# ffreyer/MonteCarlo.jl

Measured on AMD Instinct MI355X. Metric: DQMC sweeps/sec, 16x16 Hubbard beta=8 dtau=0.1; achieved % fp64 MFMA roofline, higher is better.
Workload: dtype f64

## Files before the change

montecarlo.jl_amd/csrc/engine.cpp:

```cpp
#include <hip/hip_runtime.h>

#include <algorithm>
#include <cmath>
#include <cstdio>
#include <cstdlib>
#include <cstring>
#include <string>
#include <vector>

#include "../../include/dqmc_hip.h"
#include "kernels.h"
#include "state_blob.h"
#include <rccl/rccl.h>

using namespace dqmc;

struct dqmc_comm {
    ncclComm_t comm = nullptr;
    int nranks = 1, rank = 0, device = 0;
};

static thread_local std::string g_create_error;

struct UTStack;
// ... 463 lines not shown
    auto apply = [&](int op, const double *F) {
        for (int c = 0; c < n; ++c) {
            const double *m = M.data() + (size_t)n * c;
            double *t = T.data() + (size_t)n * c;
            for (int y = 0; y < 16; ++y)
                for (int x = 0; x < 16; ++x) {
                    double acc = 0.0;
                    for (int k = 0; k < 16; ++k) {
                        const double f = F[(op == 0 ? x : y) + 16 * k];
                        const int src = op == 0 ? k + 16 * y : op == 1 ? x + 16 * k : op == 2 ? ((x - y + k) & 15) + 16 * k
                                                                                               : ((x + y - k) & 15) + 16 * k;
                        acc += f * m[src];
                    }
                    t[x + 16 * y] = acc;
                }
        }
        M.swap(T);
    };
    const double *F[4] = {fx, fy, fd, fa};
    static const int orders[5][4] = {{3, 2, 0, 1}, {1, 2, 3, 0}, {0, 2, 3, 1}, {0, 3, 2, 1}, {1, 3, 2, 0}};
    double emax = 0.0, rmax = 0.0;
    for (size_t i = 0; i < (size_t)n * n; ++i) emax = std::max(emax, std::fabs(E[i]));
    for (const auto &ord : orders) {
        std::fill(M.begin(), M.end(), 0.0);
        for (int i = 0; i < n; ++i) M[i + (size_t)n * i] = 1.0;
        for (int k = 0; k < 4; ++k) apply(ord[k], F[ord[k]]);
        for (size_t i = 0; i < (size_t)n * n; ++i) {
            const double r = std::fabs(E[i] - M[i]);
            if (!(r <= rmax)) rmax = r;
        }
    }
    return std::isfinite(emax) && std::isfinite(rmax) && rmax <= 256.0 * 2.220446049250313e-16 * emax;
}

static void read_kernel_switches(dqmc_handle *h)
{
    KernelSwitches &k = h->sw;
    k.qr_noblocked = getenv("DQMC_QR_NOBLOCKED") != nullptr;
    if (const char *e = getenv("DQMC_QRB_SITES")) k.qrb_sites = atoi(e) & 7;
    if (const char *e = getenv("DQMC_QR_TAIL")) k.qr_tail = atoi(e) != 0;
    k.qr_sc1 = getenv("DQMC_QR_SC1") != nullptr;
    k.qr_nocoop = getenv("DQMC_QR_NOCOOP") != nullptr;
    if (const char *e = getenv("DQMC_QR_FORCE_TIMEOUT"))
        k.qr_force_timeout = strncmp(e, "step:", 5) == 0 ? 2 + atoi(e + 5) : (strncmp(e, "extra:", 6) == 0 ? 1000 + atoi(e + 6) : 1);
    k.qr_nopanel = getenv("DQMC_QR_NOPANEL") != nullptr;
    k.trsm_simple = getenv("DQMC_TRSM_SIMPLE") != nullptr;
    k.sweep_split = getenv("DQMC_SWEEP_SPLIT") != nullptr;
    k.flush_ncp2 = getenv("DQMC_FLUSH_NCP2") != nullptr;
    k.no_slab = getenv("DQMC_NO_SLAB") != nullptr;
    k.no_kron = getenv("DQMC_NO_KRON") != nullptr;
    k.no_wrap_flush = getenv("DQMC_NO_WRAP_FLUSH") != nullptr;
    k.wrap_two_launch = getenv("DQMC_WRAP_TWO_LAUNCH") != nullptr;
    k.tdm_general = getenv("DQMC_TDM_GENERAL") != nullptr;
}

static int padded_units(const dqmc_handle *h) { return (h->units + 7) / 8 * 8; }
static bool udt_blocked_fits(const dqmc_handle *h, int per_cu) { return per_cu >= 1 && padded_units(h) * 8 <= h->cus * per_cu; }
static bool sweep_fused_fits(const dqmc_handle *h)
{
    const int ncp = (h->n % 256 == 0) ? 2 : 1, nt = (h->n % 128 == 0) ? 8 : 4;
    const int flush_blocks = padded_units(h) * (h->n / 64) * (h->n / (16 * nt * ncp));
    return h->W + flush_blocks <= h->cus;
}

static int alloc_qr_workspace(dqmc_handle *h)
{
    CHK(dalloc(h, &h->qr_ws.errflag, (size_t)1));
    h->qr_ws.tail = h->sw.qr_tail;
    h->qr_ws.force_sc1 = h->sw.qr_sc1;
    h->qr_ws.no_coop = h->sw.qr_nocoop;
    h->qr_ws.no_panel = h->sw.qr_nopanel;
    h->qr_ws.force_timeout = h->sw.qr_force_timeout;
    if (h->n > 256) return 0;
    hipDeviceProp_t prop;
    HIPCHK(hipGetDeviceProperties(&prop, h->p.device_id));
    h->cus = prop.multiProcessorCount;
    const size_t slots = (size_t)((h->units + 7) / 8) * 8 * QR_COOP_SLOTS_PER_UNIT;
    CHK(dalloc(h, &h->qr_ws.mailbox, slots * QR_COOP_SLOT));
    CHK(dalloc(h, &h->qr_ws.fb, (size_t)2));
    h->qr_ws.max_blocks = h->cus * qr_coop_blocks_per_cu();
    h->qr_ws.epoch = 0;
    h->qrb_sites = 0;
    if (h->n == 256 && !h->sw.qr_noblocked) {
        const int per_cu = qrb_blocks_per_cu();
        if (udt_blocked_fits(h, per_cu)) {
            CHK(dalloc(h, (char **)&h->qr_ws.mailbox2, qrb_mailbox_bytes(h->units)));
            h->qr_ws.blk_max_blocks = h->cus * per_cu;
            h->qrb_sites = h->sw.qrb_sites;
        }
    }
    return 0;
}
static int alloc_wrap_handoff(dqmc_handle *h)
{
    if (!h->kron || h->n != 256 || h->rect || h->sw.wrap_two_launch) return 0;
    hipDeviceProp_t prop;
    HIPCHK(hipGetDeviceProperties(&prop, h->p.device_id));
    h->cus = prop.multiProcessorCount;
    for (int pf = 0; pf < 2; ++pf) h->wrap_blocks[pf] = h->cus * kron_wrap_blocks_per_cu(pf != 0);
    if (kron_wrap_grid(h->units) > std::max(h->wrap_blocks[0], h->wrap_blocks[1])) return 0;
    return dalloc(h, &h->wrap_cnt, (size_t)kron_wrap_grid(h->units) / 16 * KR_CNT_STRIDE);
}
static bool wrap_one_launch(const dqmc_handle *h, bool pending)
{
    return h->wrap_cnt && h->n == 256 && !h->tri && !h->rect && kron_wrap_grid(h->units) <= h->wrap_blocks[pending ? 1 : 0];
}
// ... 28 lines not shown
        Timed t(h, DQMC_K_QR);
        HIPCHK(launch_qr_pivot(n, h->units, A, h->nn, q.tau, q.pivot, &h->qr_ws, q.W, h->nn, &F, h->stream, q.V, h->nn));
    }
    {
        Timed t(h, DQMC_K_MISC);
        HIPCHK(launch_udt_finish(n, h->units, A, h->nn, F, h->nn, q.pivot, Dout, n, q.V, h->nn, Tout, h->nn, apply,
                                 h->stream));
    }
    return 0;
}
static int udt_formq(dqmc_handle *h, double *Uout, QrSet &q)
{
    const int n = h->n;
    GemmArgs g = gemm_base(h, U_(h, q.V), 1, U_(h, q.V), 0, q.S);
    g.tri = (n % 64 == 0) ? 1 : 0;
    CHK(run_gemm(h, g));
    {
        Timed t(h, DQMC_K_TRSM);
        HIPCHK(launch_trsm_right_upper(n, h->units, q.V, h->nn, q.S, h->nn, nullptr, q.tau, n, q.W, h->nn, q.winv, h->sw, h->stream, q.ts));
    }
    g = gemm_base(h, U_(h, q.W), 0, U_(h, q.V), 1, Uout);
    g.alpha = -1.0;
    g.ident = 1.0;
    g.tri = (n % 64 == 0) ? 2 : 0;
    CHK(run_gemm(h, g));
    return 0;
}
static bool udt_is_fused(const dqmc_handle *h, int site) { return (h->qrb_sites >> site) & 1; }
static int udt_fused(dqmc_handle *h, const double *A, double *Uout, double *Dout, double *Tout, int apply, QrSet &q,
                     const double *B = nullptr)
{
    Timed t(h, DQMC_K_QR);
    HIPCHK(launch_udt_blocked(h->units, A, h->nn, Uout, h->nn, Dout, h->n, Tout, h->nn, q.pivot, &h->qr_ws, apply, h->stream, B,
                              h->nn));
    return 0;
}
static int udt(dqmc_handle *h, double *A, double *Uout, double *Dout, double *Tout, int apply)
{
    if (udt_is_fused(h, 0) && Tout && Tout != A) return udt_fused(h, A, Uout, Dout, Tout, apply, h->qs);
    CHK(udt_factor(h, A, Dout, Tout, apply, h->qs));
    return udt_formq(h, Uout, h->qs);
}
static int rdivp_set(dqmc_handle *h, const double *A, const double *T, double *Out, const QrSet &q)
{
    Timed t(h, DQMC_K_TRSM);
    HIPCHK(launch_trsm_right_upper(h->n, h->units, A, h->nn, T, h->nn, q.pivot, nullptr, 0, Out, h->nn, q.winv, h->sw, h->stream, q.ts));
    return 0;
}
static int rdivp(dqmc_handle *h, double *A, const double *T)
{
    return rdivp_set(h, A, T, A, h->qs);
}

static int calculate_greens_src(dqmc_handle *h, double *out, Udt L, Udt R, double *a2_copy = nullptr)
{
    const int n = h->n;
    QrSet &q = h->qs;
    GemmArgs g = gemm_base(h, U_(h, L.t), 0, U_(h, R.t), 1, out);
    g.colscale = vs_arr(R.d, n);
    g.rowscale = vs_arr(L.d, n);
    CHK(run_gemm(h, g));
    if (udt_is_fused(h, 1)) {
        if (L.u == h->Tl) return fail(h, DQMC_ERR_STATE, "calculate_greens: Ul aliases Tl");
        CHK(udt_fused(h, out, h->Tl, h->Dr, q.W, 0, q, L.u));
        CHK(rdivp_set(h, R.u, q.W, h->Ur, q));
    } else {
        CHK(udt_factor(h, out, h->Dr, nullptr, 0, q));
        CHK(rdivp_set(h, R.u, out, h->Ur, q));
        CHK(udt_formq(h, h->Tr, q));
        CHK(run_gemm(h, gemm_base(h, U_(h, L.u), 0, U_(h, h->Tr), 0, h->Tl)));
    }
    g = gemm_base(h, U_(h, h->Tl), 1, U_(h, h->Ur), 0, h->Tr);
    g.adddiag = vs_arr(h->Dr, n);
    CHK(run_gemm(h, g));
    if (a2_copy) CHK(copy_mat(h, a2_copy, h->Tr));
    const double *tlul = h->Tr;
    if (udt_is_fused(h, 2)) {
        CHK(udt_fused(h, h->Tr, h->Ul, h->Dr, q.W, 0, q, h->Tl));
        CHK(rdivp_set(h, h->Ur, q.W, h->Ur, q));
        tlul = h->Ul;
    } else {
        CHK(udt_factor(h, h->Tr, h->Dr, nullptr, 0, q));
        CHK(rdivp_set(h, h->Ur, h->Tr, h->Ur, q));
        CHK(udt_formq(h, h->Ul, q));
        CHK(run_gemm(h, gemm_base(h, U_(h, h->Tl), 0, U_(h, h->Ul), 0, h->Tr)));
    }
    g = gemm_base(h, U_(h, h->Ur), 0, U_(h, tlul), 1, out);
    g.kscale = vs_inv(h->Dr, n);
    CHK(run_gemm(h, g));
    return 0;
}
static int calculate_greens(dqmc_handle *h, double *out, double *a2_copy = nullptr)
{
    return calculate_greens_src(h, out, Udt{h->Ul, h->Dl, h->Tl}, Udt{h->Ur, h->Dr, h->Tr}, a2_copy);
}

enum { CB_LEFT_B = 0, CB_LEFT_BINV = 1, CB_LEFT_BDAG = 2, CB_RIGHT_B = 3, CB_RIGHT_BINV = 4, CB_RIGHT_ET = 5,
       CB_LEFT_ETINV = 6 };
static int cb_mult(dqmc_handle *h, int which, int slice, const double *X, double *O, const double *qscale)
{
    CbArgs a{};
    a.n = h->n; a.nb = h->nb; a.kmax = h->cb.kmax;
    a.side = (which == CB_RIGHT_B || which == CB_RIGHT_BINV || which == CB_RIGHT_ET) ? 1 : 0;
    a.seq_len = h->cb.len[which];
    for (int i = 0; i < a.seq_len; ++i) a.seq[i] = h->cb.seq[which][i];
    a.vals = h->cb.vals; a.cols = h->cb.cols;
    a.X = X; a.O = O; a.strideX = h->nn;
    a.conf = slice >= 1 ? h->conf + (long)(slice - 1) * h->N : nullptr;
    a.conf_stride = (long)h->N * h->M;
    a.epl = h->epl; a.eml = h->eml;
    switch (which) {
    case CB_LEFT_B: a.pre_conf = +1; a.pre_vec = h->cb.mu; break;
    case CB_LEFT_BINV: a.post_conf = -1; a.post_vec = h->cb.mu_inv; break;
    case CB_LEFT_BDAG: a.post_conf = +1; a.post_vec = h->cb.mu; break;
    case CB_RIGHT_B: a.post_conf = +1; a.post_vec = h->cb.mu; break;
    case CB_RIGHT_BINV: a.pre_conf = -1; a.pre_vec = h->cb.mu_inv; break;
    default: break;
    }
    a.qscale = qscale; a.qstride = h->n;
    hipEvent_t ea, eb;
    timing_events(h, &ea, &eb);
    HIPCHK(launch_cb_apply(a, h->units, h->stream, ea, eb));
    return timing_push(h, ea, eb, DQMC_K_GEMM);
}

static SlabArgs slab_base(dqmc_handle *h, const double *X0, long x_su, long x_sb, double *out)
{
    SlabArgs a{};
    a.n_units = h->units; a.nb = h->nb; a.nsteps = 0;
    a.X0 = X0; a.x_su = x_su; a.x_sb = x_sb;
    a.out = out; a.out_su = h->nn;
    a.conf_stride = (long)h->N * h->M;
    a.epl = h->epl; a.eml = h->eml;
    return a;
}
static void slab_step_const(dqmc_handle *h, SlabArgs &a, const double *C)
{
    SlabStep &st = a.st[a.nsteps++];
    st = SlabStep{};
    st.A = C; st.su = 0; st.sb = h->nn;
}
static void slab_step_unit(dqmc_handle *h, SlabArgs &a, const double *A)
// ... 191 lines not shown
    const int8_t *c = conf_slice(h, curr_slice);
    SlabArgs a = slab_base(h, h->eTinv2, 0, h->nn, dst);
    slab_step_unit(h, a, src);
    a.st[0].pre_conf = c; a.st[0].pre_sign = -1;
    slab_step_const(h, a, h->eT2);
    a.st[1].pre_conf = c; a.st[1].pre_sign = +1;
    return run_slab(h, a);
}
static int wrap_greens_inplace(dqmc_handle *h, double *gf, int curr_slice, int direction);
static int wrap_greens(dqmc_handle *h, double **gf, int curr_slice, int direction)
{
    if (oop_wrap(h)) {
        CHK(wrap_greens_slab(h, *gf, h->tmp1, curr_slice, direction));
        std::swap(*gf, h->tmp1);
        return 0;
    }
    return wrap_greens_inplace(h, *gf, curr_slice, direction);
}
static int wrap_greens_inplace(dqmc_handle *h, double *gf, int curr_slice, int direction)
{
    if (h->cb.on) {
        const int l = direction == -1 ? curr_slice - 1 : curr_slice;
        CHK(cb_mult(h, direction == -1 ? CB_LEFT_BINV : CB_LEFT_B, l, gf, gf, nullptr));
        CHK(cb_mult(h, direction == -1 ? CB_RIGHT_B : CB_RIGHT_BINV, l, gf, gf, nullptr));
        return 0;
    }
    if (direction == -1) {
        const int l = curr_slice - 1;
        GemmArgs g = gemm_base(h, C_(h, h->eTinv2), 0, U_(h, gf), 0, h->tmp1);
        g.rowscale = vs_conf(h, l, -1);
        CHK(run_gemm(h, g));
        g = gemm_base(h, U_(h, h->tmp1), 0, C_(h, h->eT2), 0, gf);
        g.colscale = vs_conf(h, l, +1);
        CHK(run_gemm(h, g));
    } else {
        const int l = curr_slice;
        GemmArgs g = gemm_base(h, C_(h, h->eT2), 0, U_(h, gf), 0, h->tmp1);
        g.kscale = vs_conf(h, l, +1);
        CHK(run_gemm(h, g));
        g = gemm_base(h, U_(h, h->tmp1), 0, C_(h, h->eTinv2), 0, gf);
        g.kscale = vs_conf(h, l, -1);
        CHK(run_gemm(h, g));
    }
    return 0;
}

static int reset_slot(dqmc_handle *h, int slot)
{
    const int sp = h->K + 1;
    CHK(set_identity(h, uslot(h, sp)));
    CHK(set_ones(h, dslot(h, sp)));
    CHK(set_identity(h, tslot(h, sp)));
    slot_swap_spare(h, slot);
    return 0;
}
static int prop_check(dqmc_handle *h)
{
    Timed t(h, DQMC_K_MISC);
    HIPCHK(launch_prop_check(h->n, h->nb, h->W, h->greens_temp, h->greens, h->nn, h->stats, h->pc_scratch, h->stream));
    return 0;
}

static int init_stack(dqmc_handle *h)
{
    CHK(set_identity(h, h->Ul)); CHK(set_identity(h, h->Ur));
    CHK(set_identity(h, h->Tl)); CHK(set_identity(h, h->Tr));
    CHK(set_ones(h, h->Dl)); CHK(set_ones(h, h->Dr));
    h->current_slice = 0;
    h->direction = 0;
    return 0;
}
static int build_stack(dqmc_handle *h)
{
    CHK(reset_slot(h, 0));
    for (int i = 1; i <= h->K; ++i) CHK(add_slice_sequence_left(h, i));
    h->current_slice = h->M + 1;
    h->direction = -1;
    return 0;
}

static int propagate(dqmc_handle *h)
{
    const int M = h->M, s = h->s;
    if (h->direction == 1) {
        if (h->current_slice % s == 0) {
            h->current_slice += 1;
            if (h->current_slice == 1) {
                const Udt R = slot_ref(h, 0);
                CHK(reset_slot(h, 0));
                discard_pending_flush(h);
                CHK(calculate_greens_src(h, h->greens, slot_ref(h, 0), R));
            } else if (1 < h->current_slice && h->current_slice <= M) {
                const int idx = (h->current_slice - 1) / s;
                const Udt R = slot_ref(h, idx);
                const bool wt = h->p.check_propagation_error != 0, wt_slab = wt && oop_wrap(h);
                CHK(add_slice_sequence_left(h, idx, wt_slab));
                const Udt L = slot_ref(h, idx);
                if (wt && !wt_slab) {
                    CHK(materialize_pending_flush(h));
                    CHK(copy_mat(h, h->greens_temp, h->greens));
                    CHK(wrap_greens(h, &h->greens_temp, h->current_slice - 1, 1));
                }
                if (wt_slab) {
                    std::swap(h->greens, h->greens_alt);
                    CHK(calculate_greens_src(h, h->greens, L, R));
                    CHK(prop_check(h));
                    return 0;
                }
                discard_pending_flush(h);
                CHK(calculate_greens_src(h, h->greens, L, R));
                if (h->p.check_propagation_error) CHK(prop_check(h));
            } else {
                CHK(add_slice_sequence_left(h, h->K));
                h->direction = -1;
                h->current_slice = M + 1;
                CHK(propagate(h));
            }
        } else {
            CHK(wrap_greens(h, &h->greens, h->current_slice, 1));
            h->current_slice += 1;
        }
    } else {
        if ((h->current_slice - 1) % s == 0) {
            h->current_slice -= 1;
            if (h->current_slice == M) {
                const Udt L = slot_ref(h, h->K);
                CHK(reset_slot(h, h->K));
                discard_pending_flush(h);
                CHK(calculate_greens_src(h, h->greens, L, slot_ref(h, h->K)));
                CHK(wrap_greens(h, &h->greens, h->current_slice + 1, -1));
            } else if (0 < h->current_slice && h->current_slice < M) {
                const int idx = h->current_slice / s + 1;
                const Udt L = slot_ref(h, idx - 1);
                CHK(add_slice_sequence_right(h, idx));
                const Udt R = slot_ref(h, idx - 1);
                if (h->p.check_propagation_error) {
                    CHK(materialize_pending_flush(h));
                    std::swap(h->greens_temp, h->greens);
                }
                discard_pending_flush(h);
                CHK(calculate_greens_src(h, h->greens, L, R));
                if (h->p.check_propagation_error) CHK(prop_check(h));
                CHK(wrap_greens(h, &h->greens, h->current_slice + 1, -1));
            } else {
                CHK(add_slice_sequence_right(h, 1));
                h->direction = 1;
                h->current_slice = 0;
                CHK(propagate(h));
            }
        } else {
            CHK(wrap_greens(h, &h->greens, h->current_slice, -1));
            h->current_slice -= 1;
        }
    }
    return 0;
}

static int sweep_spatial_launches(dqmc_handle *h);
static bool sweep_takes_fused(const dqmc_handle *h) { return h->sweep_fused && h->n % 64 == 0 && h->N >= 128; }
static int sweep_spatial(dqmc_handle *h)
{
    const int l = h->current_slice;
    if (l < 1 || l > h->M) return fail(h, DQMC_ERR_STATE, "sweep_spatial: current_slice outside 1..slices");
    CHK(sweep_spatial_launches(h));
    return 0;
}
static int sweep_spatial_launches(dqmc_handle *h)
{
    const int l = h->current_slice;
    int8_t *cslice = h->conf + (long)(l - 1) * h->N;
    h->conf_version++;
    CHK(materialize_pending_flush(h));
    double *cur = h->greens, *alt = h->greens_alt;
    const size_t istr = (size_t)h->units * sweep_lu_image_doubles();

    const long cstr = (long)h->N * h->M;
    hipEvent_t a, b;
    if (sweep_takes_fused(h)) {
        const int nc = h->N / 64;
        timing_events(h, &a, &b);
        HIPCHK(launch_sweep_lu(h->n, h->nb, h->W, cur, h->nn, cslice, cstr, 0, 64, h->lu_img, h->sc, h->rng, h->stats,
                               h->p.check_sign_problem, h->qr_ws.errflag, h->stream, a, b));
        CHK(timing_push(h, a, b, DQMC_K_SWEEP));
        for (int c = 1; c < nc; ++c) {
            timing_events(h, &a, &b);
            HIPCHK(launch_sweep_fused(h->n, h->nb, h->W, cur, alt, h->nn, cslice, cstr, 64 * c, 64 * (c - 1),
                                      h->lu_img + (size_t)(c & 1) * istr, h->lu_img + (size_t)((c - 1) & 1) * istr, h->sc,
                                      h->rng, h->stats, h->p.check_sign_problem, h->qr_ws.errflag, h->stream, a, b));
            CHK(timing_push(h, a, b, DQMC_K_SWEEP));
            std::swap(cur, alt);
        }
        const double *img_last = h->lu_img + (size_t)((nc - 1) & 1) * istr;
        if (fold_wrap_flush(h)) {
            h->pf = dqmc_handle::PendingFlush{cur, img_last, 64 * (nc - 1)};
        } else {
// ... 1395 lines not shown
```

montecarlo.jl_amd/csrc/kernels.h:

```cpp
#pragma once
#include <hip/hip_runtime.h>
#include <stdint.h>

namespace dqmc {

struct VecSrc {
    int mode;
    const double *d;
    long stride;
    const int8_t *conf;
    long conf_stride;
    double cpos[2], cneg[2];
};
static inline VecSrc vs_none() { VecSrc v = {}; v.mode = 0; return v; }
static inline VecSrc vs_arr(const double *d, long stride) { VecSrc v = {}; v.mode = 1; v.d = d; v.stride = stride; return v; }
static inline VecSrc vs_inv(const double *d, long stride) { VecSrc v = {}; v.mode = 3; v.d = d; v.stride = stride; return v; }
static inline VecSrc vs_min1(const double *d, long stride) { VecSrc v = {}; v.mode = 4; v.d = d; v.stride = stride; return v; }
static inline VecSrc vs_maxinv(const double *d, long stride) { VecSrc v = {}; v.mode = 5; v.d = d; v.stride = stride; return v; }
#ifdef __HIPCC__
__device__ __forceinline__ double vs_get(const VecSrc &v, int unit, int nb, int i)
{
    if (v.mode == 1) return v.d[(long)unit * v.stride + i];
    if (v.mode == 3) return 1.0 / v.d[(long)unit * v.stride + i];
    if (v.mode == 2) {
// ... 43 lines not shown
    const int8_t *col_conf; int col_sign;
    long conf_stride;
    double epl, eml;
};
hipError_t launch_slab_chain(const SlabArgs &a, hipStream_t s, hipEvent_t start = nullptr, hipEvent_t stop = nullptr);
struct KronStep {
    const double *ax, *ay;
    const int8_t *pre_conf; int pre_sign;
    const int8_t *post_conf; int post_sign;
};
struct KronArgs {
    int n_units, nb, nsteps;
    KronStep st[SLAB_MAX_STEPS];
    const double *X0; long x_su;
    double *out; long out_su;
    const double *col_d; long col_stride;
    int transpose_out;
    long conf_stride;
    double epl, eml;
    const double *pf_img; long pf_img_su;
    int pf_site0;
    double *wrap_out;
    unsigned *wrap_cnt; unsigned wrap_target;
    int *errflag;
};
hipError_t launch_kron_chain(const KronArgs &a, hipStream_t s, hipEvent_t start = nullptr, hipEvent_t stop = nullptr);
constexpr int KR_CNT_STRIDE = 32;
inline int kron_wrap_grid(int n_units) { return (n_units + 7) / 8 * 8 * 16; }
int kron_wrap_blocks_per_cu(bool pending);
hipError_t launch_kron_wrap(const KronArgs &a, hipStream_t s, hipEvent_t start = nullptr, hipEvent_t stop = nullptr);
hipError_t launch_kron3_chain(const KronArgs &a, hipStream_t s, hipEvent_t start = nullptr, hipEvent_t stop = nullptr);
hipError_t launch_tri_chain(const KronArgs &a, hipStream_t s, hipEvent_t start = nullptr, hipEvent_t stop = nullptr);
hipError_t launch_ttp_chain(const KronArgs &a, hipStream_t s, hipEvent_t start = nullptr, hipEvent_t stop = nullptr);
constexpr int BILAYER_FB = 264;
hipError_t launch_bilayer_chain(const KronArgs &a, hipStream_t s, hipEvent_t start = nullptr, hipEvent_t stop = nullptr);
hipError_t launch_rect_chain(const KronArgs &a, hipStream_t s, hipEvent_t start = nullptr, hipEvent_t stop = nullptr);

struct KernelSwitches {
    bool qr_noblocked = false;
    int qrb_sites = 7;
    bool qr_tail = true;
    bool qr_sc1 = false;
    bool qr_nocoop = false;
    int qr_force_timeout = 0;
    bool qr_nopanel = false;
    bool trsm_simple = false;
    bool sweep_split = false;
    bool flush_ncp2 = false;
    bool no_slab = false;
    bool no_kron = false;
    bool no_wrap_flush = false;
    bool wrap_two_launch = false;
    bool tdm_general = false;
};

constexpr int QR_COOP_SLOT = 528;
constexpr int QR_COOP_SLOTS_PER_UNIT = 16;
struct QrCoopWorkspace {
    double *mailbox = nullptr;
    int *errflag = nullptr;
    int *fb = nullptr;
    unsigned long long epoch = 0;
    int max_blocks = 0;
    bool tail = true;
    int force_sc1 = 0;
    int no_coop = 0;
    bool no_panel = false;
    int force_timeout = 0;
    double *mailbox2 = nullptr;
    int blk_max_blocks = 0;
};
hipError_t launch_udt_blocked(int n_units, const double *A, long strideA, double *U, long strideU, double *D, long strideD,
                              double *T, long strideT, int *pivot, QrCoopWorkspace *ws, int apply_pivot, hipStream_t s,
                              const double *B = nullptr, long strideB = 0);
size_t qrb_mailbox_bytes(int n_units);
int qrb_blocks_per_cu();
hipError_t launch_qr_pivot(int n, int n_units, double *A, long strideA, double *tau, int *pivot,
                           QrCoopWorkspace *ws, double *W, long strideW, const double **factored, hipStream_t s,
                           double *X = nullptr, long strideX = 0);
int qr_coop_blocks_per_cu();
int qr_coop_grid(int n, int n_units, const QrCoopWorkspace *ws);

hipError_t launch_udt_finish(int n, int n_units, double *A, long strideA, const double *F, long strideF,
                             const int *pivot, double *D, long strideD, double *V, long strideV, double *Tout,
                             long strideT, int apply_pivot, hipStream_t s);

hipError_t launch_trsm_right_upper(int n, int n_units, const double *A, long strideA, const double *T,
                                   long strideT, const int *pivot, const double *dmul, long strideV,
                                   double *Out, long strideOut, double *winv, const KernelSwitches &sw,
                                   hipStream_t s, double *scratch = nullptr);

struct SweepConsts {
    double gamma[2], ebos[2], dup[2], ddn[2];
};
struct WalkerRng {
    unsigned long long seed;
    unsigned long long draw;
    const double *uniforms;
    unsigned long long n_uniforms;
    int exhausted;
};
struct DevMagStats { double max, min, sum; long long count; };
struct DevStats {
    long long prop_local, acc_local;
    DevMagStats negative_probability, propagation_error;
};
#ifdef __HIPCC__
__device__ __forceinline__ double philox_uniform(unsigned long long seed, unsigned long long index)
{
    unsigned int c0 = (unsigned int)index, c1 = (unsigned int)(index >> 32), c2 = 0u, c3 = 0u;
    unsigned int k0 = (unsigned int)seed, k1 = (unsigned int)(seed >> 32);
#pragma unroll
    for (int r = 0; r < 10; ++r) {
        const unsigned long long p0 = (unsigned long long)0xD2511F53u * c0;
        const unsigned long long p1 = (unsigned long long)0xCD9E8D57u * c2;
        const unsigned int n0 = (unsigned int)(p1 >> 32) ^ c1 ^ k0;
        const unsigned int n1 = (unsigned int)p1;
        const unsigned int n2 = (unsigned int)(p0 >> 32) ^ c3 ^ k1;
        const unsigned int n3 = (unsigned int)p0;
        c0 = n0; c1 = n1; c2 = n2; c3 = n3;
        k0 += 0x9E3779B9u;
        k1 += 0xBB67AE85u;
    }
    const unsigned long long hi = c0 >> 5, lo = c1 >> 6;
    return (double)((hi << 26) | lo) * (1.0 / 9007199254740992.0);
}

__device__ __forceinline__ double philox4_uniform(unsigned long long seed, unsigned int c0, unsigned int c1,
                                                  unsigned int c2, unsigned int c3)
{
    unsigned int k0 = (unsigned int)seed, k1 = (unsigned int)(seed >> 32);
#pragma unroll
    for (int r = 0; r < 10; ++r) {
        const unsigned long long p0 = (unsigned long long)0xD2511F53u * c0;
        const unsigned long long p1 = (unsigned long long)0xCD9E8D57u * c2;
        const unsigned int n0 = (unsigned int)(p1 >> 32) ^ c1 ^ k0;
        const unsigned int n1 = (unsigned int)p1;
        const unsigned int n2 = (unsigned int)(p0 >> 32) ^ c3 ^ k1;
        const unsigned int n3 = (unsigned int)p0;
        c0 = n0; c1 = n1; c2 = n2; c3 = n3;
        k0 += 0x9E3779B9u;
        k1 += 0xBB67AE85u;
    }
// ... 199 lines not shown
```

montecarlo.jl_amd/csrc/qr.hip:

```cpp
#include "kernels.h"
#include <cstdlib>

namespace dqmc {

__device__ __forceinline__ double wave_sum(double x)
{
#pragma unroll
    for (int off = 32; off > 0; off >>= 1) x += __shfl_xor(x, off, 64);
    return x;
}

constexpr int QR_THREADS = 1024;
constexpr int QR_WAVES = QR_THREADS / 64;

template <int QMAX, int QR_UC>
__global__ __launch_bounds__(QR_THREADS) void qr_pivot_kernel(int n, double *__restrict__ Aall, long strideA,
                                                             double *__restrict__ tauall,
                                                             int *__restrict__ pivall,
                                                             const double *__restrict__ srcall, long strideSrc,
                                                             int *guard, int guard_val)
{
    extern __shared__ __attribute__((aligned(16))) double sm[];
    if (guard && guard[0] != guard_val) return;
    if (srcall) {
// ... 1686 lines not shown
}

__global__ __launch_bounds__(16) void trsm_diag_inv_kernel(int n, const double *__restrict__ Tall, long sT,
                                                          const double *__restrict__ dmulall, long sV,
                                                          double *__restrict__ Wall, int nblk)
{
    __shared__ double B[16][17], rdg[16];
    const int J = blockIdx.x, unit = blockIdx.y, j = threadIdx.x, j0 = J << 4;
    const double *__restrict__ T = Tall + (long)unit * sT;
    const double *__restrict__ dmul = dmulall ? dmulall + (long)unit * sV : nullptr;
    double *__restrict__ W = Wall + ((long)unit * nblk + J) * 256;
    const int col = j0 + j;
    {
        const int cc = min(col, n - 1);
        double bv[16], dv;
#pragma unroll
        for (int i = 0; i < 16; ++i) bv[i] = T[min(j0 + i, n - 1) + (long)n * cc];
        dv = dmul ? dmul[cc] : T[cc + (long)n * cc];
        asm volatile("" ::: "memory");
#pragma unroll
        for (int i = 0; i < 16; ++i) B[i][j] = (col < n && j0 + i < n && i < j) ? bv[i] : 0.0;
        rdg[j] = col < n ? (dmul ? dv : 1.0 / dv) : 1.0;
    }
    __syncthreads();
    double wcol[16];
#pragma unroll
    for (int i = 15; i >= 0; --i) {
        double sum = (i == j) ? 1.0 : 0.0;
#pragma unroll
        for (int kk = i + 1; kk < 16; ++kk) sum -= B[i][kk] * ((kk <= j) ? wcol[kk] : 0.0);
        wcol[i] = (i <= j) ? sum * rdg[i] : 0.0;
    }
#pragma unroll
    for (int i = 0; i < 16; ++i) W[i + 16 * j] = wcol[i];
}

__global__ void trsm_gather_kernel(int n, const double *__restrict__ Aall, long sA, const int *__restrict__ pivall,
                                   double *__restrict__ Wall, long sW)
{
    const int unit = blockIdx.y;
    const double *__restrict__ A = Aall + (long)unit * sA;
    double *__restrict__ W = Wall + (long)unit * sW;
    const int *__restrict__ piv = pivall ? pivall + (long)unit * n : nullptr;
    const long nn = (long)n * n;
    for (long idx = blockIdx.x * (long)blockDim.x + threadIdx.x; idx < nn; idx += (long)gridDim.x * blockDim.x) {
        const int r = (int)(idx % n), c = (int)(idx / n);
        W[idx] = A[r + (long)n * (piv ? piv[c] : c)];
    }
}

hipError_t launch_trsm_rl(int nr, int nc, int c0, int ld, int nblk_all, int n_units, const double *A, long sA,
                          const double *T, long sT, const int *pivot, double *Out, long sO, const double *winv,
                          hipStream_t s);

hipError_t launch_trsm_right_upper(int n, int n_units, const double *A, long sA, const double *T, long sT,
                                   const int *pivot, const double *dmul, long sV, double *Out, long sO,
                                   double *winv, const KernelSwitches &sw, hipStream_t s, double *scratch)
{
    const bool no_mfma = sw.trsm_simple;
    if (n <= 256 && winv && !no_mfma) {
        const int nblk = (n + 15) / 16;
        hipLaunchKernelGGL(trsm_diag_inv_kernel, dim3(nblk, n_units), dim3(16), 0, s, n, T, sT, dmul, sV, winv, nblk);
        return launch_trsm_rl(n, n, 0, n, nblk, n_units, A, sA, T, sT, pivot, Out, sO, winv, s);
    }
    if (n > 256 && winv && scratch && sA == sO && !no_mfma) {
        const int nblk = (n + 15) / 16;
        int pw = 256;
        for (int cand = 256; cand >= 128; cand -= 16)
            if (n % cand == 0) { pw = cand; break; }
        hipLaunchKernelGGL(trsm_diag_inv_kernel, dim3(nblk, n_units), dim3(16), 0, s, n, T, sT, dmul, sV, winv, nblk);
        int bx = (int)(((long)n * n + 255) / 256);
        if (bx > 128) bx = 128;
        hipLaunchKernelGGL(trsm_gather_kernel, dim3(bx, n_units), dim3(256), 0, s, n, A, sA, pivot, scratch, sO);
        for (int c0 = 0; c0 < n; c0 += pw) {
            const int nc = n - c0 < pw ? n - c0 : pw;
            if (c0 > 0) {
                GemmArgs g{};
                g.M = n; g.N = nc; g.K = c0;
                g.n_units = n_units; g.nb = 1;
                g.A = mat(scratch, sO, n);
                g.B = mat(T + (long)n * c0, sT, n);
                g.C = scratch + (long)n * c0; g.strideC = sO; g.ldc = n;
                g.kscale = g.colscale = g.rowscale = g.adddiag = vs_none();
                g.alpha = -1.0; g.ident = 0.0; g.beta = 1;
                hipError_t e = launch_gemm(g, s);
                if (e != hipSuccess) return e;
            }
            hipError_t er = launch_trsm_rl(n, nc, c0, n, nblk, n_units, scratch, sO, T, sT, nullptr, scratch, sO, winv, s);
            if (er != hipSuccess) return er;
        }
        hipError_t e = hipMemcpyAsync(Out, scratch, sizeof(double) * (size_t)n_units * sO, hipMemcpyDeviceToDevice, s);
        if (e != hipSuccess) return e;
        return hipGetLastError();
    }
    const size_t budget = 150 * 1024;
    auto need = [&](int rs) { return ((size_t)n * rs + ((n + 63) & ~63) + 256) * sizeof(double); };
    int rs = 64;
    while (rs > 16 && need(rs) > budget) rs >>= 1;
    if (need(rs) > budget) return hipErrorInvalidValue;
    const int slabs = (n + rs - 1) / rs;
    dim3 grid(n_units * slabs), block(256);
    const size_t lds = need(rs);
#define TR_LAUNCH(RS)                                                                                         \
    do {                                                                                                      \
        (void)hipFuncSetAttribute((const void *)trsm_kernel<RS>, hipFuncAttributeMaxDynamicSharedMemorySize, (int)lds); \
        hipLaunchKernelGGL((trsm_kernel<RS>), grid, block, lds, s, n, A, sA, T, sT, pivot, dmul, sV, Out, sO, slabs); \
// ... 10 lines not shown
```

montecarlo.jl_amd/csrc/trsm_rl.hip:

```cpp
#include "kernels.h"
#include <type_traits>

namespace dqmc {

typedef double d4_t __attribute__((ext_vector_type(4)));

#ifdef TR_STAMPS
__device__ long long *tr_stamp_ptr = nullptr;
#define TR_STAMP(idx)                                                                                        \
    do {                                                                                                     \
        if (blockIdx.x == 0 && (threadIdx.x & 63) == 0 && tr_stamp_ptr)                                      \
            tr_stamp_ptr[(threadIdx.x >> 6) * 64 + (idx)] = (long long)__builtin_amdgcn_s_memtime();         \
    } while (0)
#else
#define TR_STAMP(idx) do { } while (0)
#endif
constexpr int TR_TS = 18;
template <bool FULLB>
__global__ __launch_bounds__(256) void trsm_rl_kernel(int nr, int n, int c0, int ld, int nblk_all,
                                                     const double *__restrict__ Aall, long sA,
                                                     const double *__restrict__ Tall, long sT,
                                                     const int *__restrict__ pivall, double *__restrict__ Oall, long sO,
                                                     int slabs, const double *__restrict__ Wall, int n_units)
{
    extern __shared__ __attribute__((aligned(16))) double trl_sm[];
    double (*Tl)[256 * TR_TS] = reinterpret_cast<double (*)[256 * TR_TS]>(trl_sm);
    double (*Xi)[2][4 * 64] = reinterpret_cast<double (*)[2][4 * 64]>(trl_sm + 3 * 256 * TR_TS);
    double (*Wl)[4 * 64] = reinterpret_cast<double (*)[4 * 64]>(trl_sm + 3 * 256 * TR_TS + 2 * 2 * 256);
    const int bid = blockIdx.x, xcd = bid & 7, seq = bid >> 3;
    const int unit = (seq / slabs) * 8 + xcd, row0 = (seq % slabs) * 32;
    if (unit >= n_units) return;
    const double *__restrict__ A = Aall + (long)unit * sA;
    const double *__restrict__ T = Tall + (long)unit * sT + (long)ld * c0 + c0;
    const int *__restrict__ piv = pivall ? pivall + (long)unit * ld : nullptr;
    double *__restrict__ O = Oall + (long)unit * sO;
    const int tid = threadIdx.x, lane = tid & 63, w = tid >> 6, g = lane >> 4, ci = lane & 15;
    const int rt = w & 1, par = w >> 1;
    const int nblk = FULLB ? 16 : (n + 15) >> 4;
    const double *__restrict__ Wu = Wall + ((long)unit * nblk_all + (c0 >> 4)) * 256;
    const int row = row0 + 16 * rt + ci;
    const int rowc = min(row, nr - 1);

    TR_STAMP(0);
    d4_t x[8];
    int pjv[8][4];
#pragma unroll
    for (int t = 0; t < 8; ++t)
#pragma unroll
        for (int r = 0; r < 4; ++r) {
            const int cc = min(16 * (2 * t + par) + 4 * r + g, n - 1);
            pjv[t][r] = piv ? piv[c0 + cc] : c0 + cc;
        }
#pragma unroll
    for (int t = 0; t < 8; ++t)
#pragma unroll
        for (int r = 0; r < 4; ++r) x[t][r] = A[(unsigned)(rowc + ld * pjv[t][r])];
    asm volatile("" ::: "memory");
#pragma unroll
    for (int t = 0; t < 8; ++t) {
        const int L = 2 * t + par;
#pragma unroll
        for (int r = 0; r < 4; ++r) {
            const int col = 16 * L + 4 * r + g;
            x[t][r] = (L < nblk && col < n && row < nr) ? x[t][r] : 0.0;
        }
    }
#ifdef TR_STAMPS
    TR_STAMP(40);
    asm volatile("s_waitcnt vmcnt(0)" ::: "memory");
    TR_STAMP(41);
#endif
    constexpr int TR_RING = 3;
    double pv[TR_RING][16];
    auto request = [&](auto Jc) {
        constexpr int J = decltype(Jc)::value, S = J % TR_RING;
        if (J >= nblk) return;
        const int k = FULLB ? 16 * J + (tid & 15) : min(16 * J + (tid & 15), n - 1);
#pragma unroll
        for (int i = (FULLB ? J + 1 : 0); i < 16; ++i) {
            const int c = FULLB ? (tid >> 4) + 16 * i : min((tid >> 4) + 16 * i, n - 1);
            pv[S][i] = T[(unsigned)(ld * c + k)];
        }
    };
    auto deposit = [&](auto Jc) {
        constexpr int J = decltype(Jc)::value, S = J % TR_RING;
        if (J >= nblk) return;
        double *tl = Tl[J % 3];
        const int k = tid & 15;
#pragma unroll
        for (int i = (FULLB ? J + 1 : 0); i < 16; ++i) {
            const int c = (tid >> 4) + 16 * i;
            const bool live = FULLB || (c < n && c >= 16 * (J + 1) && 16 * J + k < n);
            tl[c * TR_TS + k] = live ? pv[S][i] : 0.0;
        }
    };
    auto finish = [&](auto Jc) {
        constexpr int J = decltype(Jc)::value, t_own = J >> 1;
        d4_t o = {0.0, 0.0, 0.0, 0.0};
#pragma unroll
        for (int q = 0; q < 4; ++q) o = __builtin_amdgcn_mfma_f64_16x16x4f64(Wl[J][q * 64 + lane], x[t_own][q], o, 0, 0, 0);
#pragma unroll
        for (int r = 0; r < 4; ++r) {
            Xi[J & 1][rt][r * 64 + lane] = o[r];
            const int col = 16 * J + 4 * r + g;
            if (FULLB || (row < nr && col < n)) O[(unsigned)(row + ld * (c0 + col))] = o[r];
        }
    };
#define TRL_IC(K) std::integral_constant<int, (K)>{}
    request(TRL_IC(0));
    request(TRL_IC(1));
    request(TRL_IC(2));
    {
        const int q = tid >> 6, l = tid & 63, src = (4 * q + (l >> 4)) + 16 * (l & 15);
        double wv[16];
#pragma unroll
        for (int J = 0; J < 16; ++J) wv[J] = Wu[(unsigned)((FULLB ? J : min(J, nblk - 1)) * 256 + src)];
#pragma unroll
        for (int J = 0; J < 16; ++J) Wl[J][tid] = wv[J];
    }
#ifdef TR_STAMPS
    TR_STAMP(42);
    asm volatile("s_waitcnt vmcnt(0)" ::: "memory");
    TR_STAMP(43);
#endif
    deposit(TRL_IC(0));
    TR_STAMP(44);
    __syncthreads();
    TR_STAMP(1);
    if (par == 0) finish(TRL_IC(0));
    deposit(TRL_IC(1));
    request(TRL_IC(3));
    asm volatile("s_waitcnt lgkmcnt(0)\n\ts_barrier" ::: "memory");
    auto step = [&](auto Jc) {
        constexpr int J = decltype(Jc)::value;
        if (!FULLB && J >= nblk) return;
        const double *xi = Xi[J & 1][rt];
        const double *tl = Tl[J % 3];
        const double b0 = -xi[lane], b1 = -xi[64 + lane], b2 = -xi[128 + lane], b3 = -xi[192 + lane];
        auto body = [&](auto pc) {
            constexpr int PAR = decltype(pc)::value;
            constexpr bool own_next = J + 1 < 16 && ((J + 1) & 1) == PAR;
            constexpr int t_next = (J + 1) >> 1;
            if constexpr (own_next) {
                if (FULLB || J + 1 < nblk) {
                    const double *ta = tl + (16 * (J + 1) + ci) * TR_TS + g;
                    x[t_next] = __builtin_amdgcn_mfma_f64_16x16x4f64(ta[0], b0, x[t_next], 0, 0, 0);
                    x[t_next] = __builtin_amdgcn_mfma_f64_16x16x4f64(ta[4], b1, x[t_next], 0, 0, 0);
                    x[t_next] = __builtin_amdgcn_mfma_f64_16x16x4f64(ta[8], b2, x[t_next], 0, 0, 0);
                    x[t_next] = __builtin_amdgcn_mfma_f64_16x16x4f64(ta[12], b3, x[t_next], 0, 0, 0);
                    finish(TRL_IC(J + 1 < 16 ? J + 1 : 15));
                }
            }
            constexpr int t_first = own_next ? t_next + 1 : (J + 2 - PAR) / 2;
            const double bq[4] = {b0, b1, b2, b3};
#pragma unroll
            for (int q = 0; q < 4; ++q)
#pragma unroll
                for (int t = t_first; t < 8; ++t) {
                    if (!FULLB && 2 * t + PAR >= nblk) continue;
                    const double *ta = tl + (16 * (2 * t + PAR) + ci) * TR_TS + g;
                    x[t] = __builtin_amdgcn_mfma_f64_16x16x4f64(ta[4 * q], bq[q], x[t], 0, 0, 0);
                }
        };
        if (par == 0) body(TRL_IC(0));
        else body(TRL_IC(1));
        deposit(TRL_IC(J + 2));
        request(TRL_IC(J + 4));
        TR_STAMP(2 + 2 * J);
        asm volatile("s_waitcnt lgkmcnt(0)\n\ts_barrier" ::: "memory");
        TR_STAMP(3 + 2 * J);
    };
#define TRL_STEP(K) step(std::integral_constant<int, K>{})
    TRL_STEP(0); TRL_STEP(1); TRL_STEP(2); TRL_STEP(3); TRL_STEP(4); TRL_STEP(5); TRL_STEP(6); TRL_STEP(7);
    TRL_STEP(8); TRL_STEP(9); TRL_STEP(10); TRL_STEP(11); TRL_STEP(12); TRL_STEP(13); TRL_STEP(14); TRL_STEP(15);
#undef TRL_STEP
#undef TRL_IC
    TR_STAMP(34);
}
#ifdef TR_STAMPS
extern "C" int dqmc_debug_tr_stamps(void *devptr)
{
    return (int)hipMemcpyToSymbol(HIP_SYMBOL(tr_stamp_ptr), &devptr, sizeof(void *));
}
#endif

hipError_t launch_trsm_rl(int nr, int nc, int c0, int ld, int nblk_all, int n_units, const double *A, long sA,
                          const double *T, long sT, const int *pivot, double *Out, long sO, const double *winv,
                          hipStream_t s)
{
    if (nc > 256 || nc < 1) return hipErrorInvalidValue;
    const size_t lds_r = (3 * 256 * TR_TS + 2 * 2 * 256 + 16 * 256) * sizeof(double);
    int dev = 0;
    (void)hipGetDevice(&dev);
    static unsigned attr_mask = 0;
    if (!(attr_mask & (1u << dev))) {
        (void)hipFuncSetAttribute((const void *)trsm_rl_kernel<true>, hipFuncAttributeMaxDynamicSharedMemorySize, (int)lds_r);
        (void)hipFuncSetAttribute((const void *)trsm_rl_kernel<false>, hipFuncAttributeMaxDynamicSharedMemorySize, (int)lds_r);
        attr_mask |= 1u << dev;
    }
    const int slabs = (nr + 31) / 32;
    const int groups = (n_units + 7) / 8;
    if (nc == 256 && nr % 32 == 0)
        hipLaunchKernelGGL(trsm_rl_kernel<true>, dim3(groups * 8 * slabs), dim3(256), lds_r, s, nr, nc, c0, ld, nblk_all, A, sA, T,
                           sT, pivot, Out, sO, slabs, winv, n_units);
    else
        hipLaunchKernelGGL(trsm_rl_kernel<false>, dim3(groups * 8 * slabs), dim3(256), lds_r, s, nr, nc, c0, ld, nblk_all, A, sA,
                           T, sT, pivot, Out, sO, slabs, winv, n_units);
    return hipGetLastError();
}

}
```

Baseline: 821.1.

## Fuse right triangular solve with final Green's product and propagation check

For n=256, the last rdivp triangular solve of calculate_greens is fused with the closing GEMM (Ur·diag(1/D)·(TlUl)^T) and, when requested, the propagation-error check, all in one kernel. The solved slab stays in registers and LDS instead of being written to Ur and read back by a separate GEMM and check kernel. This removes two launches and a full matrix round trip per Green's function. The cost is a more complex kernel with extra register pressure, and a product phase that reuses the T-panel LDS region.

```diff
diff --git a/montecarlo.jl_amd/csrc/engine.cpp b/montecarlo.jl_amd/csrc/engine.cpp
--- a/montecarlo.jl_amd/csrc/engine.cpp
+++ b/montecarlo.jl_amd/csrc/engine.cpp
@@ -539,6 +539,8 @@
     k.no_wrap_flush = getenv("DQMC_NO_WRAP_FLUSH") != nullptr;
     k.wrap_two_launch = getenv("DQMC_WRAP_TWO_LAUNCH") != nullptr;
     k.tdm_general = getenv("DQMC_TDM_GENERAL") != nullptr;
+    k.no_rdivp_product = getenv("DQMC_NO_RDIVP_PRODUCT") != nullptr;
+    k.no_rdivp_check = getenv("DQMC_NO_RDIVP_CHECK") != nullptr;
 }
 
 static int padded_units(const dqmc_handle *h) { return (h->units + 7) / 8 * 8; }
@@ -673,7 +675,18 @@
     return rdivp_set(h, A, T, A, h->qs);
 }
 
-static int calculate_greens_src(dqmc_handle *h, double *out, Udt L, Udt R, double *a2_copy = nullptr)
+static int prop_check(dqmc_handle *h, const double *A, const double *B)
+{
+    Timed t(h, DQMC_K_MISC);
+    HIPCHK(launch_prop_check(h->n, h->nb, h->W, A, B, h->nn, h->stats, h->pc_scratch, h->stream));
+    return 0;
+}
+static bool rdivp_product_on(const dqmc_handle *h)
+{
+    return h->n == 256 && !h->sw.no_rdivp_product && !h->sw.trsm_simple && h->qs.winv;
+}
+static int calculate_greens_src(dqmc_handle *h, double *out, Udt L, Udt R, double *a2_copy = nullptr,
+                                const double *check = nullptr)
 {
     const int n = h->n;
     QrSet &q = h->qs;
@@ -696,19 +709,38 @@
     CHK(run_gemm(h, g));
     if (a2_copy) CHK(copy_mat(h, a2_copy, h->Tr));
     const double *tlul = h->Tr;
+    const double *t2 = h->Tr;
+    const bool fused = rdivp_product_on(h);
     if (udt_is_fused(h, 2)) {
         CHK(udt_fused(h, h->Tr, h->Ul, h->Dr, q.W, 0, q, h->Tl));
-        CHK(rdivp_set(h, h->Ur, q.W, h->Ur, q));
+        if (!fused) CHK(rdivp_set(h, h->Ur, q.W, h->Ur, q));
         tlul = h->Ul;
+        t2 = q.W;
+    } else if (fused) {
+        CHK(udt_factor(h, h->Tr, h->Dr, nullptr, 0, q));
+        CHK(udt_formq(h, h->Ul, q));
+        CHK(run_gemm(h, gemm_base(h, U_(h, h->Tl), 0, U_(h, h->Ul), 0, q.W)));
+        tlul = q.W;
     } else {
         CHK(udt_factor(h, h->Tr, h->Dr, nullptr, 0, q));
         CHK(rdivp_set(h, h->Ur, h->Tr, h->Ur, q));
         CHK(udt_formq(h, h->Ul, q));
         CHK(run_gemm(h, gemm_base(h, U_(h, h->Tl), 0, U_(h, h->Ul), 0, h->Tr)));
     }
+    if (fused) {
+        const bool in_launch = check && !h->sw.no_rdivp_check;
+        {
+            Timed t(h, DQMC_K_TRSM);
+            HIPCHK(launch_rdivp_product(n, h->units, h->Ur, h->nn, t2, h->nn, q.pivot, q.winv, tlul, h->nn, h->Dr, n, out, h->nn,
+                                        in_launch ? check : nullptr, h->stats, h->pc_scratch, h->nb, h->stream));
+        }
+        if (check && !in_launch) CHK(prop_check(h, check, out));
+        return 0;
+    }
     g = gemm_base(h, U_(h, h->Ur), 0, U_(h, tlul), 1, out);
     g.kscale = vs_inv(h->Dr, n);
     CHK(run_gemm(h, g));
+    if (check) CHK(prop_check(h, check, out));
     return 0;
 }
 static int calculate_greens(dqmc_handle *h, double *out, double *a2_copy = nullptr)
@@ -1006,12 +1038,6 @@
     CHK(set_ones(h, dslot(h, sp)));
     CHK(set_identity(h, tslot(h, sp)));
     slot_swap_spare(h, slot);
-    return 0;
-}
-static int prop_check(dqmc_handle *h)
-{
-    Timed t(h, DQMC_K_MISC);
-    HIPCHK(launch_prop_check(h->n, h->nb, h->W, h->greens_temp, h->greens, h->nn, h->stats, h->pc_scratch, h->stream));
     return 0;
 }
 
@@ -1057,13 +1083,11 @@
                 }
                 if (wt_slab) {
                     std::swap(h->greens, h->greens_alt);
-                    CHK(calculate_greens_src(h, h->greens, L, R));
-                    CHK(prop_check(h));
+                    CHK(calculate_greens_src(h, h->greens, L, R, nullptr, h->greens_temp));
                     return 0;
                 }
                 discard_pending_flush(h);
-                CHK(calculate_greens_src(h, h->greens, L, R));
-                if (h->p.check_propagation_error) CHK(prop_check(h));
+                CHK(calculate_greens_src(h, h->greens, L, R, nullptr, h->p.check_propagation_error ? h->greens_temp : nullptr));
             } else {
                 CHK(add_slice_sequence_left(h, h->K));
                 h->direction = -1;
@@ -1093,8 +1117,7 @@
                     std::swap(h->greens_temp, h->greens);
                 }
                 discard_pending_flush(h);
-                CHK(calculate_greens_src(h, h->greens, L, R));
-                if (h->p.check_propagation_error) CHK(prop_check(h));
+                CHK(calculate_greens_src(h, h->greens, L, R, nullptr, h->p.check_propagation_error ? h->greens_temp : nullptr));
                 CHK(wrap_greens(h, &h->greens, h->current_slice + 1, -1));
             } else {
                 CHK(add_slice_sequence_right(h, 1));
diff --git a/montecarlo.jl_amd/csrc/kernels.h b/montecarlo.jl_amd/csrc/kernels.h
--- a/montecarlo.jl_amd/csrc/kernels.h
+++ b/montecarlo.jl_amd/csrc/kernels.h
@@ -119,6 +119,8 @@
     bool no_wrap_flush = false;
     bool wrap_two_launch = false;
     bool tdm_general = false;
+    bool no_rdivp_product = false;
+    bool no_rdivp_check = false;
 };
 
 constexpr int QR_COOP_SLOT = 528;
@@ -156,6 +158,12 @@
                                    long strideT, const int *pivot, const double *dmul, long strideV,
                                    double *Out, long strideOut, double *winv, const KernelSwitches &sw,
                                    hipStream_t s, double *scratch = nullptr);
+
+struct DevStats;
+hipError_t launch_rdivp_product(int n, int n_units, const double *A, long strideA, const double *T, long strideT,
+                                const int *pivot, double *winv, const double *B, long strideB, const double *D,
+                                long strideD, double *C, long strideC, const double *Gt, DevStats *stats,
+                                unsigned long long *pc_scratch, int nb, hipStream_t s);
 
 struct SweepConsts {
     double gamma[2], ebos[2], dup[2], ddn[2];
diff --git a/montecarlo.jl_amd/csrc/qr.hip b/montecarlo.jl_amd/csrc/qr.hip
--- a/montecarlo.jl_amd/csrc/qr.hip
+++ b/montecarlo.jl_amd/csrc/qr.hip
@@ -1762,6 +1762,19 @@
 hipError_t launch_trsm_rl(int nr, int nc, int c0, int ld, int nblk_all, int n_units, const double *A, long sA,
                           const double *T, long sT, const int *pivot, double *Out, long sO, const double *winv,
                           hipStream_t s);
+
+hipError_t launch_trsm_rl_product(int n_units, const double *A, long sA, const double *T, long sT, const int *pivot,
+                                  const double *winv, const double *B, long sB, const double *D, long sD, double *C, long sC,
+                                  const double *Gt, DevStats *stats, unsigned long long *pc_scratch, int nb, hipStream_t s);
+
+hipError_t launch_rdivp_product(int n, int n_units, const double *A, long sA, const double *T, long sT, const int *pivot,
+                                double *winv, const double *B, long sB, const double *D, long sD, double *C, long sC,
+                                const double *Gt, DevStats *stats, unsigned long long *pc_scratch, int nb, hipStream_t s)
+{
+    if (n != 256 || !winv) return hipErrorInvalidValue;
+    hipLaunchKernelGGL(trsm_diag_inv_kernel, dim3(16, n_units), dim3(16), 0, s, n, T, sT, (const double *)nullptr, 0l, winv, 16);
+    return launch_trsm_rl_product(n_units, A, sA, T, sT, pivot, winv, B, sB, D, sD, C, sC, Gt, stats, pc_scratch, nb, s);
+}
 
 hipError_t launch_trsm_right_upper(int n, int n_units, const double *A, long sA, const double *T, long sT,
                                    const int *pivot, const double *dmul, long sV, double *Out, long sO,
diff --git a/montecarlo.jl_amd/csrc/trsm_rl.hip b/montecarlo.jl_amd/csrc/trsm_rl.hip
--- a/montecarlo.jl_amd/csrc/trsm_rl.hip
+++ b/montecarlo.jl_amd/csrc/trsm_rl.hip
@@ -16,13 +16,24 @@
 #define TR_STAMP(idx) do { } while (0)
 #endif
 constexpr int TR_TS = 18;
-template <bool FULLB>
-__global__ __launch_bounds__(256) void trsm_rl_kernel(int nr, int n, int c0, int ld, int nblk_all,
-                                                     const double *__restrict__ Aall, long sA,
-                                                     const double *__restrict__ Tall, long sT,
-                                                     const int *__restrict__ pivall, double *__restrict__ Oall, long sO,
-                                                     int slabs, const double *__restrict__ Wall, int n_units)
-{
+struct RdivpProd {
+    const double *B; long sB;
+    const double *D; long sD;
+    double *C; long sC;
+    const double *Gt;
+    DevStats *stats;
+    unsigned long long *pc;
+    int nb;
+};
+constexpr int RP_RING = 4;
+template <bool FULLB, int PROD>
+__device__ __forceinline__ void trsm_rl_body(int nr, int n, int c0, int ld, int nblk_all,
+                                             const double *__restrict__ Aall, long sA,
+                                             const double *__restrict__ Tall, long sT,
+                                             const int *__restrict__ pivall, double *__restrict__ Oall, long sO,
+                                             int slabs, const double *__restrict__ Wall, int n_units, const RdivpProd &pr)
+{
+    static_assert(PROD == 0 || FULLB, "the product phase exists for whole 256-column slabs only");
     extern __shared__ __attribute__((aligned(16))) double trl_sm[];
     double (*Tl)[256 * TR_TS] = reinterpret_cast<double (*)[256 * TR_TS]>(trl_sm);
     double (*Xi)[2][4 * 64] = reinterpret_cast<double (*)[2][4 * 64]>(trl_sm + 3 * 256 * TR_TS);
@@ -103,8 +114,10 @@
         for (int r = 0; r < 4; ++r) {
             Xi[J & 1][rt][r * 64 + lane] = o[r];
             const int col = 16 * J + 4 * r + g;
+            if (PROD) continue;
             if (FULLB || (row < nr && col < n)) O[(unsigned)(row + ld * (c0 + col))] = o[r];
         }
+        if (PROD) x[t_own] = o;
     };
 #define TRL_IC(K) std::integral_constant<int, (K)>{}
     request(TRL_IC(0));
@@ -172,11 +185,139 @@
     };
 #define TRL_STEP(K) step(std::integral_constant<int, K>{})
     TRL_STEP(0); TRL_STEP(1); TRL_STEP(2); TRL_STEP(3); TRL_STEP(4); TRL_STEP(5); TRL_STEP(6); TRL_STEP(7);
-    TRL_STEP(8); TRL_STEP(9); TRL_STEP(10); TRL_STEP(11); TRL_STEP(12); TRL_STEP(13); TRL_STEP(14); TRL_STEP(15);
+    TRL_STEP(8); TRL_STEP(9); TRL_STEP(10); TRL_STEP(11);
+    const double *__restrict__ Bu = PROD ? pr.B + (long)unit * pr.sB : nullptr;
+    double dk[8][4], av[RP_RING][4], gt[PROD == 2 ? 8 : 1][4];
+    auto request_b = [&](auto kc) {
+        constexpr int kg = decltype(kc)::value;
+        if constexpr (kg < 64) {
+#pragma unroll
+            for (int j = 0; j < 4; ++j) av[kg % RP_RING][j] = Bu[(unsigned)(16 * (4 * w + j) + ci + ld * (4 * kg + g))];
+        }
+    };
+    if constexpr (PROD != 0) {
+        const double *__restrict__ Du = pr.D + (long)unit * pr.sD;
+#pragma unroll
+        for (int t = 0; t < 8; ++t)
+#pragma unroll
+            for (int r = 0; r < 4; ++r) dk[t][r] = Du[16 * (2 * t + par) + 4 * r + g];
+    }
+    TRL_STEP(12); TRL_STEP(13);
+    if constexpr (PROD != 0) {
+        request_b(TRL_IC(0)); request_b(TRL_IC(1)); request_b(TRL_IC(2)); request_b(TRL_IC(3));
+    }
+    TRL_STEP(14);
+    if constexpr (PROD == 0) {
+        TRL_STEP(15);
+    } else {
+        TR_STAMP(34);
+        double *img = trl_sm;
+#pragma unroll
+        for (int t = 0; t < 8; ++t)
+#pragma unroll
+            for (int r = 0; r < 4; ++r) img[((2 * t + par) * 2 + rt) * 256 + r * 64 + lane] = x[t][r] * (1.0 / dk[t][r]);
+        asm volatile("s_waitcnt lgkmcnt(0)\n\ts_barrier" ::: "memory");
+        TR_STAMP(35);
+        d4_t acc[4][2];
+#pragma unroll
+        for (int j = 0; j < 4; ++j) acc[j][0] = acc[j][1] = (d4_t){0.0, 0.0, 0.0, 0.0};
+        const double *__restrict__ Gu = PROD == 2 ? pr.Gt + (long)unit * pr.sC : nullptr;
+        auto group = [&](auto kc) {
+            constexpr int kg = decltype(kc)::value;
+            const double b0 = img[((kg >> 2) * 2 + 0) * 256 + (kg & 3) * 64 + lane];
+            const double b1 = img[((kg >> 2) * 2 + 1) * 256 + (kg & 3) * 64 + lane];
+            double a[4];
+#pragma unroll
+            for (int j = 0; j < 4; ++j) a[j] = av[kg % RP_RING][j];
+#pragma unroll
+            for (int j = 0; j < 4; ++j) {
+                acc[j][0] = __builtin_amdgcn_mfma_f64_16x16x4f64(a[j], b0, acc[j][0], 0, 0, 0);
+                acc[j][1] = __builtin_amdgcn_mfma_f64_16x16x4f64(a[j], b1, acc[j][1], 0, 0, 0);
+            }
+            request_b(TRL_IC(kg + RP_RING));
+            if constexpr (PROD == 2 && kg == 64 - RP_RING - 1) {
+#pragma unroll
+                for (int j = 0; j < 4; ++j)
+#pragma unroll
+                    for (int u = 0; u < 2; ++u)
+#pragma unroll
+                        for (int r = 0; r < 4; ++r)
+                            gt[2 * j + u][r] = Gu[(unsigned)(row0 + 16 * u + ci + ld * (16 * (4 * w + j) + 4 * r + g))];
+            }
+        };
+#define TRL_G4(K) group(TRL_IC(K)); group(TRL_IC(K + 1)); group(TRL_IC(K + 2)); group(TRL_IC(K + 3))
+        TRL_G4(0); TRL_G4(4); TRL_G4(8); TRL_G4(12); TRL_G4(16); TRL_G4(20); TRL_G4(24); TRL_G4(28);
+        TRL_G4(32); TRL_G4(36); TRL_G4(40); TRL_G4(44); TRL_G4(48); TRL_G4(52); TRL_G4(56); TRL_G4(60);
+#undef TRL_G4
+        TR_STAMP(36);
+        double *__restrict__ Cu = pr.C + (long)unit * pr.sC;
+        double dmax = 0.0;
+        bool bad = false;
+#pragma unroll
+        for (int j = 0; j < 4; ++j)
+#pragma unroll
+            for (int u = 0; u < 2; ++u)
+#pragma unroll
+                for (int r = 0; r < 4; ++r) {
+                    const int m = row0 + 16 * u + ci, nn = 16 * (4 * w + j) + 4 * r + g;
+                    double v = acc[j][u][r];
+                    if (m == nn) v += 0.0;
+                    Cu[(unsigned)(m + ld * nn)] = v;
+                    if constexpr (PROD == 2) {
+                        const double e = fabs(gt[2 * j + u][r] - v);
+                        bad |= (e != e);
+                        dmax = fmax(dmax, e);
+                    }
+                }
+        if constexpr (PROD == 2) {
+            const double qnan = __longlong_as_double(0x7ff8000000000000ll);
+            if (bad) dmax = qnan;
+#pragma unroll
+            for (int off = 32; off > 0; off >>= 1) {
+                const double o = __shfl_xor(dmax, off, 64);
+                dmax = (dmax != dmax || o != o) ? qnan : fmax(dmax, o);
+            }
+            double *red = trl_sm + 16 * 2 * 256;
+            if (lane == 0) red[w] = dmax;
+            __syncthreads();
+            if (tid == 0) {
+                for (int i = 1; i < 4; ++i) dmax = (dmax != dmax || red[i] != red[i]) ? qnan : fmax(dmax, red[i]);
+                const int wk = unit / pr.nb;
+                atomicMax(&pr.pc[2 * wk], (unsigned long long)__double_as_longlong(dmax));
+                __threadfence();
+                if (atomicAdd(&pr.pc[2 * wk + 1], 1ull) == (unsigned long long)(pr.nb * slabs - 1)) {
+                    __threadfence();
+                    const double mx = __longlong_as_double((long long)atomicExch(&pr.pc[2 * wk], 0ull));
+                    pr.pc[2 * wk + 1] = 0ull;
+                    if (mx > 1e-7) magstats_push(pr.stats[wk].propagation_error, mx);
+                }
+            }
+        }
+        TR_STAMP(37);
+        return;
+    }
 #undef TRL_STEP
 #undef TRL_IC
     TR_STAMP(34);
 }
+template <bool FULLB>
+__global__ __launch_bounds__(256) void trsm_rl_kernel(int nr, int n, int c0, int ld, int nblk_all,
+                                                     const double *__restrict__ Aall, long sA,
+                                                     const double *__restrict__ Tall, long sT,
+                                                     const int *__restrict__ pivall, double *__restrict__ Oall, long sO,
+                                                     int slabs, const double *__restrict__ Wall, int n_units)
+{
+    trsm_rl_body<FULLB, 0>(nr, n, c0, ld, nblk_all, Aall, sA, Tall, sT, pivall, Oall, sO, slabs, Wall, n_units, RdivpProd{});
+}
+template <int PROD>
+__global__ __launch_bounds__(256) void rdivp_product_kernel(const double *__restrict__ Aall, long sA,
+                                                           const double *__restrict__ Tall, long sT,
+                                                           const int *__restrict__ pivall, const double *__restrict__ Wall,
+                                                           int n_units, RdivpProd pr)
+{
+    static_assert(PROD == 1 || PROD == 2, "");
+    trsm_rl_body<true, PROD>(256, 256, 0, 256, 16, Aall, sA, Tall, sT, pivall, nullptr, 0, 8, Wall, n_units, pr);
+}
 #ifdef TR_STAMPS
 extern "C" int dqmc_debug_tr_stamps(void *devptr)
 {
@@ -184,29 +325,54 @@
 }
 #endif
 
-hipError_t launch_trsm_rl(int nr, int nc, int c0, int ld, int nblk_all, int n_units, const double *A, long sA,
-                          const double *T, long sT, const int *pivot, double *Out, long sO, const double *winv,
-                          hipStream_t s)
-{
-    if (nc > 256 || nc < 1) return hipErrorInvalidValue;
-    const size_t lds_r = (3 * 256 * TR_TS + 2 * 2 * 256 + 16 * 256) * sizeof(double);
+constexpr size_t TRL_LDS = (3 * 256 * TR_TS + 2 * 2 * 256 + 16 * 256) * sizeof(double);
+static_assert((16 * 2 * 256 + 4) * sizeof(double) <= 3 * 256 * TR_TS * sizeof(double), "the images of the product phase lie over the T panels");
+static void trsm_rl_attributes()
+{
     int dev = 0;
     (void)hipGetDevice(&dev);
     static unsigned attr_mask = 0;
     if (!(attr_mask & (1u << dev))) {
-        (void)hipFuncSetAttribute((const void *)trsm_rl_kernel<true>, hipFuncAttributeMaxDynamicSharedMemorySize, (int)lds_r);
-        (void)hipFuncSetAttribute((const void *)trsm_rl_kernel<false>, hipFuncAttributeMaxDynamicSharedMemorySize, (int)lds_r);
+        (void)hipFuncSetAttribute((const void *)trsm_rl_kernel<true>, hipFuncAttributeMaxDynamicSharedMemorySize, (int)TRL_LDS);
+        (void)hipFuncSetAttribute((const void *)trsm_rl_kernel<false>, hipFuncAttributeMaxDynamicSharedMemorySize, (int)TRL_LDS);
+        (void)hipFuncSetAttribute((const void *)rdivp_product_kernel<1>, hipFuncAttributeMaxDynamicSharedMemorySize, (int)TRL_LDS);
+        (void)hipFuncSetAttribute((const void *)rdivp_product_kernel<2>, hipFuncAttributeMaxDynamicSharedMemorySize, (int)TRL_LDS);
         attr_mask |= 1u << dev;
     }
+}
+
+hipError_t launch_trsm_rl(int nr, int nc, int c0, int ld, int nblk_all, int n_units, const double *A, long sA,
+                          const double *T, long sT, const int *pivot, double *Out, long sO, const double *winv,
+                          hipStream_t s)
+{
+    if (nc > 256 || nc < 1) return hipErrorInvalidValue;
+    trsm_rl_attributes();
     const int slabs = (nr + 31) / 32;
     const int groups = (n_units + 7) / 8;
     if (nc == 256 && nr % 32 == 0)
-        hipLaunchKernelGGL(trsm_rl_kernel<true>, dim3(groups * 8 * slabs), dim3(256), lds_r, s, nr, nc, c0, ld, nblk_all, A, sA, T,
+        hipLaunchKernelGGL(trsm_rl_kernel<true>, dim3(groups * 8 * slabs), dim3(256), TRL_LDS, s, nr, nc, c0, ld, nblk_all, A, sA, T,
                            sT, pivot, Out, sO, slabs, winv, n_units);
     else
-        hipLaunchKernelGGL(trsm_rl_kernel<false>, dim3(groups * 8 * slabs), dim3(256), lds_r, s, nr, nc, c0, ld, nblk_all, A, sA,
+        hipLaunchKernelGGL(trsm_rl_kernel<false>, dim3(groups * 8 * slabs), dim3(256), TRL_LDS, s, nr, nc, c0, ld, nblk_all, A, sA,
                            T, sT, pivot, Out, sO, slabs, winv, n_units);
     return hipGetLastError();
 }
 
-}
+hipError_t launch_trsm_rl_product(int n_units, const double *A, long sA, const double *T, long sT, const int *pivot,
+                                  const double *winv, const double *B, long sB, const double *D, long sD, double *C, long sC,
+                                  const double *Gt, DevStats *stats, unsigned long long *pc_scratch, int nb, hipStream_t s)
+{
+    if (!winv || !B || !D || !C || nb < 1 || (Gt && (!stats || !pc_scratch || n_units % nb != 0))) return hipErrorInvalidValue;
+    trsm_rl_attributes();
+    const int slabs = 8, groups = (n_units + 7) / 8;
+    const RdivpProd pr{B, sB, D, sD, C, sC, Gt, stats, pc_scratch, nb};
+    if (Gt)
+        hipLaunchKernelGGL(rdivp_product_kernel<2>, dim3(groups * 8 * slabs), dim3(256), TRL_LDS, s, A, sA, T, sT, pivot, winv,
+                           n_units, pr);
+    else
+        hipLaunchKernelGGL(rdivp_product_kernel<1>, dim3(groups * 8 * slabs), dim3(256), TRL_LDS, s, A, sA, T, sT, pivot, winv,
+                           n_units, pr);
+    return hipGetLastError();
+}
+
+}
```

After: 825.8, median of 6. Within noise of the previous version (+0.6%).
